# yynps737/zero-latency-yolo

Hardware: AMD Instinct MI355X
Metric: frames_per_sec (higher is better)
Workload: dtype bf16; 1 GPU; YOLOv8-nano 416x416 batch=64 throughput path (BASELINE configs[2]), bf16; engines_per_gpu=3, weights=seeded synthetic (no real weights offline), graph=True, parallelism=single GPU

## Files before the change

zero-latency-yolo_amd/csrc/engine.cpp:

```cpp
#include "zly_internal.h"
#include "weights.h"

#include <algorithm>
#include <atomic>
#include <chrono>
#include <condition_variable>
#include <deque>
#include <map>
#include <mutex>
#include <string>
#include <thread>
#include <type_traits>
#include <vector>
#include <string.h>
#include <stdio.h>
#include <stdlib.h>

namespace zly {

static thread_local std::string g_last_error;

static int fail(int code, const std::string& msg) { g_last_error = msg; return code; }

#define HIP_TRY(expr, code)                                                                        \
// ... 734 lines not shown
    }
    ca.w1 = wb + g.w1; ca.b1 = (const float*)(wb + g.b1); ca.nk1 = g.nk1;
    ca.cat = cb.ptr; ca.cat_cs = cb.C; ca.pair_in_co = e->ops[(size_t)pg.first].in.co; ca.pair_out_co = pg.out.co;
    ca.wA = wb + pg.wA; ca.bA = (const float*)(wb + pg.bA); ca.wB = wb + pg.wB; ca.bB = (const float*)(wb + pg.bB);
    ca.res = g.res;
    ca.w2 = wb + g.w2; ca.b2 = (const float*)(wb + g.b2); ca.nk2 = g.nk2; ca.Cout2 = g.cout2;
    ca.out = ob.ptr; ca.out_cs = ob.C; ca.out_co = g.out.co;
    ca.H = cb.H; ca.W = cb.W; ca.n = n;
    ca.TH = pl.th; ca.TW = pl.tw; ca.tiles_x = pl.tiles_x; ca.tiles_y = pl.tiles_y; ca.total_tiles = pl.total_tiles;
    ca.dump = (e->cfg.flags & ZLY_FLAG_DUMP_LOGITS) ? 1 : 0;
    if (g.c == 64 && g.mid.buf >= 0) { const Buffer& mb = e->bufs[(size_t)g.mid.buf]; ca.mid = mb.ptr; ca.mid_cs = mb.C; }
    return ca;
}

static const std::vector<Launch>& resolve_launches(zly_engine* e, int n)
{
    auto it = e->launches.find(n);
    if (it != e->launches.end()) return it->second;
    const bool bf16 = e->dtype == ZLY_DTYPE_BF16, fusion = bf16 && !(e->cfg.flags & ZLY_FLAG_NO_FUSION), dump = (e->cfg.flags & ZLY_FLAG_DUMP_LOGITS) != 0;
    const int nops = (int)e->ops.size();
    auto c2f_of = [&](const C2fGroup& g, C2fPlan* pl) {
        if (!fusion || e->sw.no_c2f) return false;
        const Buffer& b = e->bufs[(size_t)g.cat];
        return c2f_plan(g.c, g.mode, g.nk1, g.nk2, g.cout2, n, b.H, b.W, e->sw, pl);
    };
    auto pair_of = [&](int a, PairPlan* pl) {
        const Op& A = e->ops[(size_t)a];
        if (A.pair < 0 || !fusion) return false;
        const PairGroup& g = e->pairs[(size_t)A.pair];
        if (g.first != a || !(e->sw.pair_widths & g.c)) return false;
        const Buffer& b = e->bufs[(size_t)A.in.buf];
        return pair_plan(g.c, n, b.H, b.W, e->sw, pl) && pl->total_tiles >= e->sw.pair_min_tiles;
    };
    auto ws_pair_of = [&](int a, WsPairPlan* pl) {
        const Op& A = e->ops[(size_t)a];
        if (A.pair < 0 || !fusion) return false;
        const PairGroup& g = e->pairs[(size_t)A.pair];
        if (g.first != a || g.c != 64 || (e->sw.pair_widths & 64)) return false;
        const ConvArgs ca = make_conv_args(e, A, n), cb = make_conv_args(e, e->ops[(size_t)g.second], n);
        ConvPlan pa{}, pb{};
        conv_plan(e->dtype, 3, ca, e->sw, &pa);
        conv_plan(e->dtype, 3, cb, e->sw, &pb);
        return conv_ws_pair_plan(ca, cb, pa, pb, e->sw, pl);
    };
    bool sppf = fusion && e->sw.sppf_fused && e->sppf_cv1 >= 0;
    if (sppf) {
        const Op& a = e->ops[(size_t)e->sppf_cv1];
// ... 1824 lines not shown
```

zero-latency-yolo_amd/csrc/kernels_pair.hip:

```cpp
#include "zly_internal.h"
#include "conv_device.h"
#include <stdlib.h>
#include <stdio.h>
#include <type_traits>

namespace zly {

typedef __attribute__((ext_vector_type(4))) short s16x4;
typedef __attribute__((ext_vector_type(4))) unsigned int u32x4_t;

template <int C> struct PairGeom;
template <> struct PairGeom<16> {
    static constexpr int CT = 1, KS = 1, FRAGB = 8, PITCH = 48, WTILE = 512;
    static constexpr bool WRES = true;
    typedef s16x4 frag;
    static __device__ __forceinline__ f32x4 mma(frag a, frag b, f32x4 c) { return __builtin_amdgcn_mfma_f32_16x16x16bf16_1k(a, b, c, 0, 0, 0); }
};
template <> struct PairGeom<32> {
    static constexpr int CT = 2, KS = 1, FRAGB = 16, PITCH = 96, WTILE = 1024;
    static constexpr bool WRES = true;
    typedef bf16x8 frag;
    static __device__ __forceinline__ f32x4 mma(frag a, frag b, f32x4 c) { return __builtin_amdgcn_mfma_f32_16x16x32_bf16(a, b, c, 0, 0, 0); }
};
template <> struct PairGeom<64> {
    static constexpr int CT = 4, KS = 2, FRAGB = 16, PITCH = 160, WTILE = 1024;
    static constexpr bool WRES = false;
    typedef bf16x8 frag;
    static __device__ __forceinline__ f32x4 mma(frag a, frag b, f32x4 c) { return __builtin_amdgcn_mfma_f32_16x16x32_bf16(a, b, c, 0, 0, 0); }
};

__device__ __forceinline__ int div_small(int q, float inv) { return (int)(((float)q + 0.5f) * inv); }

template <int C>
__device__ __forceinline__ void pair_taps(const unsigned char* __restrict__ src, const unsigned char* __restrict__ lw, int off, int rowb, int lane,
                                          f32x4 (&acc)[PairGeom<C>::CT])
{
    typedef PairGeom<C> G;
    typedef typename G::frag F;
#pragma unroll
    for (int c = 0; c < G::CT; ++c) acc[c] = f32x4{0.f, 0.f, 0.f, 0.f};
    const unsigned char* wl = lw + lane * G::FRAGB;
    const int kxo[3] = {0, G::FRAGB == 8 ? opaque_offset(G::PITCH) : G::PITCH, G::FRAGB == 8 ? opaque_offset(2 * G::PITCH) : 2 * G::PITCH};
#pragma unroll
    for (int ky = 0; ky < 3; ++ky) {
        const unsigned char* row = src + off + ky * rowb;
#pragma unroll
        for (int kx = 0; kx < 3; ++kx) {
#pragma unroll
            for (int ks = 0; ks < G::KS; ++ks) {
                const F x = *reinterpret_cast<const F*>(row + (G::FRAGB == 8 ? kxo[kx] : kx * G::PITCH) + ks * 64);
#pragma unroll
                for (int c = 0; c < G::CT; ++c) {
                    const F w = *reinterpret_cast<const F*>(wl + ((c * 9 + ky * 3 + kx) * G::KS + ks) * G::WTILE);
                    acc[c] = G::mma(w, x, acc[c]);
// ... 158 lines not shown
                        }
                        store8(dst + g2 * 32 + kq * 8, lo, hi);
                    }
                }
            }
        }
        if (tnext >= a.total_tiles) break;
        tl = tnext;
        __syncthreads();
    }
}

#ifdef ZLY_C2F_DIAG
__device__ unsigned long long* g_c2f_diag = nullptr;
#define C2FSTAMP(k) do { __builtin_amdgcn_sched_barrier(0); unsigned long long t_; asm volatile("s_memtime %0\n\ts_waitcnt lgkmcnt(0)" : "=s"(t_) :: "memory"); dsum[k] += t_ - dT0; dT0 = t_; __builtin_amdgcn_sched_barrier(0); } while (0)
#else
#define C2FSTAMP(k) do { } while (0)
#endif
static constexpr int C2F_BIAS_BYTES = 1024;
static constexpr bool c2f_ring(int c, int mode) { return c == 32 && mode == 3; }
static constexpr bool c2f_y2reg(int c, int mode) { return c == 32 && (mode & 2) != 0; }
static constexpr bool c2f_tight(int c, int nw) { return c == 32 && nw == 16; }
static constexpr int C2F_MAXY = 4;
template <int C, int MODE, int NW, int NLD, int NK1>
__global__ __launch_bounds__(NW * 64) void c2f_kernel(const C2fArgs a)
{
    typedef PairGeom<C> G;
    typedef typename G::frag F;
    constexpr bool FRONT = (MODE & 1) != 0, BACK = (MODE & 2) != 0;
    constexpr bool RING = c2f_ring(C, MODE), Y2REG = c2f_y2reg(C, MODE), TIGHT = c2f_tight(C, NW);
    constexpr int NT = NW * 64;
    constexpr int UPP = C / 8;
    constexpr int WBYTES = 9 * G::CT * G::WTILE;
    constexpr int T1 = 2 * C / 16;
    constexpr int T2MAX = 4;
    extern __shared__ __attribute__((aligned(16))) unsigned char smem[];
#ifdef ZLY_C2F_DIAG
    unsigned long long dsum[12] = {0, 0, 0, 0, 0, 0, 0, 0, 0, 0, 0, 0}, dT0 = __builtin_amdgcn_s_memtime();
    const unsigned long long dstart = dT0;
#endif
    const int PW = a.TW + 4, PH = a.TH + 4, MW = a.TW + 2, MH = a.TH + 2;
    const int w1_bytes = FRONT ? T1 * a.nk1 * 1024 : 0;
    const int T2 = a.Cout2 >> 4;
    const int w2_bytes = BACK ? T2 * a.nk2 * G::WTILE : 0;
    float* lbias = reinterpret_cast<float*>(smem);
    unsigned char* lwA = smem + C2F_BIAS_BYTES;
    unsigned char* lwB = lwA + WBYTES;
    unsigned char* lw1 = lwB + WBYTES;
    unsigned char* lw2 = lw1 + w1_bytes;
    unsigned char* lin = lw2 + w2_bytes;
    unsigned char* lmid = lin + (PH * PW * G::PITCH + 15) / 16 * 16;
    unsigned char* ly2 = lmid + (MH * MW * G::PITCH + 15) / 16 * 16;
    unsigned char* ly0 = ly2 + (BACK && !Y2REG ? (a.TH * a.TW * G::PITCH + 15) / 16 * 16 : 0);

    const int tid = threadIdx.x, lane = tid & 63;
    const int wave = __builtin_amdgcn_readfirstlane(tid >> 6);
    const int p = lane & 15, kq = lane >> 4;
    bf16_t* __restrict__ cat = static_cast<bf16_t*>(a.cat);

    auto stage = [&](unsigned char* dst, const void* src, int bytes) {
        for (int u = tid; u < bytes / 16; u += NT)
            *reinterpret_cast<u32x4_t*>(dst + (size_t)u * 16) = *reinterpret_cast<const u32x4_t*>(static_cast<const unsigned char*>(src) + (size_t)u * 16);
    };
    stage(lwA, a.wA, WBYTES);
    stage(lwB, a.wB, WBYTES);
    if (FRONT) stage(lw1, a.w1, w1_bytes);
    if (BACK) stage(lw2, a.w2, w2_bytes);

    constexpr bool BIAS_LDS = C == 32 && NW == 16;
    if (BIAS_LDS) {
        for (int u = tid; u < C; u += NT) { lbias[u] = a.bA[u]; lbias[C + u] = a.bB[u]; }
        if (FRONT) for (int u = tid; u < 2 * C; u += NT) lbias[2 * C + u] = a.b1[u];
        if (BACK) for (int u = tid; u < a.Cout2; u += NT) lbias[4 * C + u] = a.b2[u];
    }
    constexpr int NBR = BIAS_LDS ? 1 : G::CT, NB1 = BIAS_LDS ? 1 : T1, NB2 = BIAS_LDS ? 1 : T2MAX;
    f32x4 rbA[NBR], rbB[NBR], rb1[NB1], rb2[NB2];
    if (!BIAS_LDS) {
#pragma unroll
        for (int c = 0; c < G::CT; ++c) {
            const int ch = C == 16 ? kq * 4 : (c >> 1) * 32 + kq * 8 + (c & 1) * 4;
            rbA[c % NBR] = *reinterpret_cast<const f32x4*>(a.bA + ch);
// ... 14 lines not shown
            return *reinterpret_cast<const f32x4*>(lbias + base + (c >> 1) * 32 + kq * 8 + (c & 1) * 4);
        }
        return which == 0 ? rbA[c % NBR] : which == 1 ? rbB[c % NBR] : which == 2 ? rb1[c % NB1] : rb2[c % NB2];
    };
    const float invPW = 1.0f / (float)PW, invMW = 1.0f / (float)MW, invTW = 1.0f / (float)a.TW;
    const int tiles_per_img = a.tiles_x * a.tiles_y;
    const int NP0 = PH * PW, NPA = MH * MW, NPB = a.TH * a.TW;
    const int ntA = (NPA + 15) >> 4, ntB = (NPB + 15) >> 4;
    const int NPR = RING ? 4 * PW + 4 * a.TH : 0;
    const int NPI = RING ? NPB : NP0;
    const int ntR = (NPR + 15) >> 4, nt0 = ntR + ((NPI + 15) >> 4);
    const int NPU = NP0 * UPP;

    auto tile_origin = [&](int tl, int& b, int& y0, int& x0) {
        b = tl / tiles_per_img;
        const int r = tl - b * tiles_per_img;
        const int ty = r / a.tiles_x;
        y0 = ty * a.TH; x0 = (r - ty * a.tiles_x) * a.TW;
    };
    auto put_map = [&](unsigned char* dst, const f32x4* o) {
        if (C == 16) store4(reinterpret_cast<bf16_t*>(dst) + kq * 4, o[0]);
        else store8(reinterpret_cast<bf16_t*>(dst) + kq * 8, o[0], o[1]);
    };
    const __amdgpu_buffer_rsrc_t rcat = __builtin_amdgcn_make_buffer_rsrc(a.cat, 0, (unsigned)((size_t)a.n * a.H * a.W * a.cat_cs * 2), 0x00020000);
    auto put_global = [&](int elem, const f32x4* o) {
        if (C == 16) {
            const bf16x4 v = to_bf16x4(o[0]);
            typedef __attribute__((ext_vector_type(2))) unsigned int u32x2_t;
            __builtin_amdgcn_raw_buffer_store_b64(__builtin_bit_cast(u32x2_t, v), rcat, (elem + kq * 4) * 2, 0, 0);
        } else {
            const bf16x8 v = to_bf16x8(o[0], o[1]);
            __builtin_amdgcn_raw_buffer_store_b128(__builtin_bit_cast(u32x4_t, v), rcat, (elem + kq * 8) * 2, 0, 0);
        }
    };

    u32x4_t pre[NLD];
    auto stage_load = [&](int tl) {
        int b, y0, x0;
        tile_origin(tl, b, y0, x0);
        const bf16_t* in = cat + a.pair_in_co;
#pragma unroll
        for (int i = 0; i < NLD; ++i) {
            const int u = tid + i * NT;
            u32x4_t v = {0u, 0u, 0u, 0u};
            if (u < NPU) {
                const int px = u / UPP, part = u - px * UPP;
                const int py = div_small(px, invPW), pxx = px - py * PW;
                const int gy = y0 - 2 + py, gx = x0 - 2 + pxx;
                if ((unsigned)gy < (unsigned)a.H && (unsigned)gx < (unsigned)a.W)
                    v = *reinterpret_cast<const u32x4_t*>(in + ((size_t)(b * a.H + gy) * a.W + gx) * a.cat_cs + part * 8);
            }
            pre[i] = v;
        }
    };
    auto stage_store = [&]() {
#pragma unroll
        for (int i = 0; i < NLD; ++i) {
            const int u = tid + i * NT;
            if (u < NPU) {
                const int px = u / UPP, part = u - px * UPP;
                *reinterpret_cast<u32x4_t*>(lin + px * G::PITCH + part * 16) = pre[i];
            }
        }
    };

    int tl = blockIdx.x;
    if (tl >= a.total_tiles) return;
    if (!FRONT) stage_load(tl);
    C2FSTAMP(0);
    while (true) {
        int b, y0, x0;
        tile_origin(tl, b, y0, x0);
        const int tnext = tl + gridDim.x;
        if (!FRONT) {
            stage_store();
            __syncthreads();
            C2FSTAMP(1);
            if (tnext < a.total_tiles) stage_load(tnext);
        } else {
            const int pF = TIGHT ? opaque_offset(p) : p, kqF = TIGHT ? opaque_offset(kq) : kq, laneF = TIGHT ? opaque_offset(lane) : lane;
            const bf16_t* __restrict__ xa = static_cast<const bf16_t*>(a.x) + a.x_co;
            const bf16_t* __restrict__ xb = static_cast<const bf16_t*>(a.x2) + a.x2_co;
            const bool dual = a.x2 != nullptr;
            const unsigned char* w1l = lw1 + laneF * 16;
            auto cv1_pixel = [&](int t, int& py, int& px) -> bool {
                if (RING && t < ntR) {
                    const int q = t * 16 + pF, r = min(q, NPR - 1);
                    if (r < 4 * PW) {
                        const int row = div_small(r, invPW);
                        px = r - row * PW; py = row < 2 ? row : row + a.TH;
                    } else {
                        const int s = r - 4 * PW, col = s & 3;
                        py = 2 + (s >> 2); px = col < 2 ? col : col + a.TW;
                    }
                    return q < NPR;
                }
                const int q = (t - ntR) * 16 + pF, j = min(q, NPI - 1);
                if (RING) {
                    const int iy = div_small(j, invTW);
                    py = iy + 2; px = j - iy * a.TW + 2;
                } else {
                    py = div_small(j, invPW); px = j - py * PW;
                }
                return q < NPI;
            };
            auto load_x = [&](int t, bf16x8 (&xf)[NK1]) {
                int py, px;
                cv1_pixel(t, py, px);
                const int gy = y0 - 2 + py, gx = x0 - 2 + px;
                const bool inimg = (unsigned)gy < (unsigned)a.H && (unsigned)gx < (unsigned)a.W;
                const size_t pa = dual ? ((size_t)(b * (a.H >> 1) + (gy >> 1)) * (a.W >> 1) + (gx >> 1)) * a.x_cs : ((size_t)(b * a.H + gy) * a.W + gx) * a.x_cs;
                const size_t pb2 = ((size_t)(b * a.H + gy) * a.W + gx) * a.x2_cs;
#pragma unroll
                for (int s = 0; s < NK1; ++s) {
                    const int ci = s * 32 + kqF * 8;
#pragma unroll
                    for (int j = 0; j < 8; ++j) xf[s][j] = (bf16_t)0.0f;
                    if (inimg) xf[s] = (dual && ci >= a.split_c) ? *reinterpret_cast<const bf16x8*>(xb + pb2 + (ci - a.split_c)) : *reinterpret_cast<const bf16x8*>(xa + pa + ci);
                }
            };
            bf16x8 xcur[NK1], xnext[NK1];
            if (wave < nt0) load_x(wave, xcur);
            __syncthreads();
            C2FSTAMP(1);
            auto cv1_tile = [&](auto c0, int t) {
                constexpr int C0 = decltype(c0)::value;
                f32x4 acc[T1];
#pragma unroll
                for (int c = C0; c < T1; ++c) acc[c] = f32x4{0.f, 0.f, 0.f, 0.f};
#pragma unroll
                for (int s = 0; s < NK1; ++s)
#pragma unroll
                    for (int c = C0; c < T1; ++c) {
                        const bf16x8 wf = *reinterpret_cast<const bf16x8*>(w1l + (c * NK1 + s) * 1024);
                        acc[c] = __builtin_amdgcn_mfma_f32_16x16x32_bf16(wf, xcur[s], acc[c], 0, 0, 0);
                    }
#pragma unroll
                for (int s = 0; s < NK1; ++s) xcur[s] = xnext[s];
                int py, px;
                const bool valid = cv1_pixel(t, py, px);
                const int gy = y0 - 2 + py, gx = x0 - 2 + px;
                const bool inimg = (unsigned)gy < (unsigned)a.H && (unsigned)gx < (unsigned)a.W;
                f32x4 o[T1];
#pragma unroll
                for (int c = C0; c < T1; ++c) {
                    f32x4 v = acc[c] + bias_of(2, c);
#pragma unroll
                    for (int r = 0; r < 4; ++r) v[r] = inimg ? silu<bf16_t>(v[r]) : 0.0f;
                    o[c] = v;
                }
                if (valid) {
                    put_map(lin + (size_t)(py * PW + px) * G::PITCH, o + G::CT);
                    if (C0 == 0 && inimg && (RING || ((unsigned)(py - 2) < (unsigned)a.TH && (unsigned)(px - 2) < (unsigned)a.TW))) {
                        if (MODE == 3) put_map(ly0 + (size_t)((py - 2) * a.TW + px - 2) * G::PITCH, o);
                        if (MODE == 1 || a.dump) {
                            const int dst = ((b * a.H + gy) * a.W + gx) * a.cat_cs;
                            put_global(dst, o);
                            put_global(dst + C, o + G::CT);
                        }
                    }
                }
            };
            for (int t = wave; t < nt0; t += NW) {
                if (t + NW < nt0) load_x(t + NW, xnext);
                if (RING && t < ntR) cv1_tile(std::integral_constant<int, G::CT>(), t);
                else cv1_tile(std::integral_constant<int, 0>(), t);
            }
            C2FSTAMP(2);
            __syncthreads();
            C2FSTAMP(3);
        }

        const int pA = TIGHT ? opaque_offset(p) : p, kqA = TIGHT ? opaque_offset(kq) : kq, laneA = TIGHT ? opaque_offset(lane) : lane;
        for (int t = wave; t < ntA; t += NW) {
            const int q = t * 16 + pA;
            const int qc = min(q, NPA - 1);
            const int my = div_small(qc, invMW), mx = qc - my * MW;
            f32x4 acc[G::CT];
            pair_taps<C>(lin, lwA, (my * PW + mx) * G::PITCH + kqA * G::FRAGB, PW * G::PITCH, laneA, acc);
            const int gy = y0 - 1 + my, gx = x0 - 1 + mx;
            const bool inimg = (unsigned)gy < (unsigned)a.H && (unsigned)gx < (unsigned)a.W;
            f32x4 o[G::CT];
#pragma unroll
            for (int c = 0; c < G::CT; ++c) {
                f32x4 v = acc[c] + bias_of(0, c);
#pragma unroll
                for (int r = 0; r < 4; ++r) v[r] = inimg ? silu<bf16_t>(v[r]) : 0.0f;
                o[c] = v;
            }
            if (q < NPA) put_map(lmid + (size_t)(my * MW + mx) * G::PITCH, o);
        }
        C2FSTAMP(4);
        __syncthreads();
        C2FSTAMP(5);

        constexpr int NS = MODE == 2 ? 4 : 3;
        const int pB = TIGHT ? opaque_offset(p) : p, kqB = TIGHT ? opaque_offset(kq) : kq, laneB = TIGHT ? opaque_offset(lane) : lane;
        constexpr int NY = Y2REG ? C2F_MAXY : 1;
        F y2f[NY], xs2[NS - 1], xs2n[NS - 1];
#pragma unroll
        for (int i = 0; i < NY; ++i) y2f[i] = F{};
#pragma unroll
        for (int s = 0; s < NS - 1; ++s) xs2n[s] = F{};
        auto y2_put = [&](int i, F v) {
            static_assert(C2F_MAXY == 4, "one branch per carried tile");
            if (i == 0) y2f[0] = v; else if (i == 1) y2f[1 % NY] = v; else if (i == 2) y2f[2 % NY] = v; else y2f[3 % NY] = v;
        };
        auto y2_get = [&](int i) -> F { return i == 0 ? y2f[0] : i == 1 ? y2f[1 % NY] : i == 2 ? y2f[2 % NY] : y2f[3 % NY]; };
        auto load_cv2 = [&](int t, F (&x)[NS - 1]) {
            const int qc = min(t * 16 + pB, NPB - 1);
            const int oy = div_small(qc, invTW), ox = qc - oy * a.TW;
            if (MODE == 2) {
                const int gy = min(y0 + oy, a.H - 1), gx = min(x0 + ox, a.W - 1);
                const bf16_t* gp = cat + ((size_t)(b * a.H + gy) * a.W + gx) * a.cat_cs + kqB * (G::FRAGB / 2);
                x[0] = *reinterpret_cast<const F*>(gp);
                x[1] = *reinterpret_cast<const F*>(gp + C);
            } else {
                x[0] = *reinterpret_cast<const F*>(ly0 + (size_t)qc * G::PITCH + kqB * G::FRAGB);
            }
            x[NS - 2] = *reinterpret_cast<const F*>(lin + (size_t)((oy + 2) * PW + ox + 2) * G::PITCH + kqB * G::FRAGB);
        };
        if (Y2REG) load_cv2(wave, xs2);
        auto conv_b_tile = [&](int t, int i) {
            if (BACK && TIGHT) asm volatile("" ::: "memory");
            const int q = t * 16 + pB;
            const int qc = min(q, NPB - 1);
            const int oy = div_small(qc, invTW), ox = qc - oy * a.TW;
            f32x4 acc[G::CT];
            pair_taps<C>(lmid, lwB, (oy * MW + ox) * G::PITCH + kqB * G::FRAGB, MW * G::PITCH, laneB, acc);
            f32x4 o[G::CT];
#pragma unroll
            for (int c = 0; c < G::CT; ++c) {
                f32x4 v = acc[c] + bias_of(1, c);
#pragma unroll
                for (int r = 0; r < 4; ++r) v[r] = silu<bf16_t>(v[r]);
                o[c] = v;
            }
            const int gy = y0 + oy, gx = x0 + ox;
            if (a.res) {
                const unsigned char* xs = lin + ((oy + 2) * PW + ox + 2) * G::PITCH;
                if (C == 16) o[0] += load4(reinterpret_cast<const bf16_t*>(xs) + kqB * 4);
                else { f32x4 ra, rb; load8(reinterpret_cast<const bf16_t*>(xs) + kqB * 8, ra, rb); o[0] += ra; o[1 % G::CT] += rb; }
            }
            if constexpr (Y2REG) {
                if constexpr (C == 16) y2_put(i, __builtin_bit_cast(F, to_bf16x4(o[0])));
                else y2_put(i, __builtin_bit_cast(F, to_bf16x8(o[0], o[1 % G::CT])));
            } else if (BACK && q < NPB) put_map(ly2 + (size_t)qc * G::PITCH, o);
            if ((!BACK || a.dump) && q < NPB && gy < a.H && gx < a.W)
                put_global(((b * a.H + gy) * a.W + gx) * a.cat_cs + a.pair_out_co, o);
        };
        for (int t = wave, i = 0; t < ntB; t += NW, ++i) conv_b_tile(t, i);

        C2FSTAMP(6);
        if (BACK) {
            if (!Y2REG) __syncthreads();
            C2FSTAMP(7);
            const unsigned char* w2l = lw2 + laneB * G::FRAGB;
            for (int t = wave, i = 0; t < ntB; t += NW, ++i) {
                if (!Y2REG) load_cv2(t, xs2);
                else if (t + NW < ntB) load_cv2(t + NW, xs2n);
                const int q = t * 16 + pB;
                const int qc = min(q, NPB - 1);
                const F yf = Y2REG ? y2_get(i) : *reinterpret_cast<const F*>(ly2 + (size_t)qc * G::PITCH + kqB * G::FRAGB);
                const int oy = div_small(qc, invTW), ox = qc - oy * a.TW;
                const int gy = min(y0 + oy, a.H - 1), gx = min(x0 + ox, a.W - 1);
                f32x4 acc[T2MAX];
#pragma unroll
                for (int c = 0; c < T2MAX; ++c) acc[c] = f32x4{0.f, 0.f, 0.f, 0.f};
#pragma unroll
                for (int s = 0; s < NS; ++s)
#pragma unroll
                    for (int c = 0; c < T2MAX; ++c)
                        if (c < T2) acc[c] = G::mma(*reinterpret_cast<const F*>(w2l + (c * NS + s) * G::WTILE), s < NS - 1 ? xs2[s < NS - 1 ? s : 0] : yf, acc[c]);
                if (Y2REG) {
#pragma unroll
                    for (int s = 0; s < NS - 1; ++s) xs2[s] = xs2n[s];
                }
                if (q < NPB && y0 + oy < a.H && x0 + ox < a.W) {
                    bf16_t* dst = static_cast<bf16_t*>(a.out) + ((size_t)(b * a.H + gy) * a.W + gx) * a.out_cs + a.out_co;
#pragma unroll
                    for (int g2 = 0; g2 < T2MAX / 2; ++g2) {
                        if (2 * g2 >= T2) break;
                        f32x4 lo = acc[2 * g2] + bias_of(3, 2 * g2), hi = acc[2 * g2 + 1] + bias_of(3, 2 * g2 + 1);
#pragma unroll
                        for (int r = 0; r < 4; ++r) { lo[r] = silu<bf16_t>(lo[r]); hi[r] = silu<bf16_t>(hi[r]); }
                        store8(dst + g2 * 32 + kqB * 8, lo, hi);
                    }
                }
            }
        }
        C2FSTAMP(8);
        if (tnext >= a.total_tiles) break;
        tl = tnext;
        if (!FRONT) __syncthreads();
    }
#ifdef ZLY_C2F_DIAG
    if (lane == 0 && g_c2f_diag) {
        unsigned long long* o = g_c2f_diag + ((size_t)blockIdx.x * NW + wave) * 16;
        for (int i = 0; i < 9; ++i) o[i] = dsum[i];
        o[9] = __builtin_amdgcn_s_memtime() - dstart;
    }
#endif
}

static constexpr int PAIR_NW16 = 16, PAIR_NW32 = 8, PAIR_NW64 = 8, PAIR_NLD = 4, PAIR_NLD64 = 6;
static int pair_nw(int c) { return c == 16 ? PAIR_NW16 : PAIR_NW32; }
static int pair_nld(int c) { return c == 64 ? PAIR_NLD64 : PAIR_NLD; }
static constexpr int PAIR_LDS_MAX = 160 * 1024;

// ... 39 lines not shown
}

static constexpr int C2F_NW16 = 16, C2F_NW32 = 8, C2F_NLD = 4;
static int c2f_nw32(int mode, const Switches& sw)
{
    if (sw.c2f32_nw == 8 || sw.c2f32_nw == 16) return sw.c2f32_nw;
    return mode == 1 ? C2F_NW32 : 16;
}
static size_t c2f_lds_bytes(int c, int mode, int nk1, int nk2, int cout2, int th, int tw)
{
    const size_t pitch = (size_t)pair_pitch(c), wtile = c == 16 ? 512 : 1024, ct = c / 16;
    size_t b = C2F_BIAS_BYTES + 2 * 9 * ct * wtile;
    if (mode & 1) b += (size_t)(2 * c / 16) * nk1 * 1024;
    if (mode & 2) b += (size_t)(cout2 / 16) * nk2 * wtile;
    b += ((size_t)(th + 4) * (tw + 4) * pitch + 15) / 16 * 16 + ((size_t)(th + 2) * (tw + 2) * pitch + 15) / 16 * 16;
    if ((mode & 2) && !c2f_y2reg(c, mode)) b += ((size_t)th * tw * pitch + 15) / 16 * 16;
    if (mode == 3) b += ((size_t)th * tw * pitch + 15) / 16 * 16;
    return b;
}

typedef void (*c2f_fn)(const C2fArgs);
static c2f_fn pick_c2f(int c, int mode, int nk1, int nw32);

bool c2f_plan(int c, int mode, int nk1, int nk2, int cout2, int n, int H, int W, const Switches& sw, C2fPlan* plan)
{
    if (c == 64 && mode >= 1 && mode <= 3) return c2f64_plan(mode, nk1, nk2, cout2, n, H, W, sw, plan);
    if ((c != 16 && c != 32) || mode < 1 || mode > 3 || !pick_c2f(c, mode, nk1, c2f_nw32(mode, sw))) return false;
    if ((mode & 2) && nk2 != (mode == 2 ? 4 : 3)) return false;
    const int ncu = sw.num_cus, nw = c == 16 ? C2F_NW16 : c2f_nw32(mode, sw);
    const size_t lds_cap = sw.c2f_lds_kb ? (size_t)sw.c2f_lds_kb * 1024 : (size_t)PAIR_LDS_MAX;
    double best = 1e30;
    for (int th = 4; th <= 32; ++th) {
        for (int tw = 8; tw <= 64; ++tw) {
            if (c2f_lds_bytes(c, mode, nk1, nk2, cout2, th, tw) > lds_cap) continue;
            if (sw.c2f_tile_th && (sw.c2f_tile_th != th || sw.c2f_tile_tw != tw)) continue;
            if (!(mode & 1) && (th + 4) * (tw + 4) * (c / 8) > nw * 64 * C2F_NLD) continue;
            if (c2f_y2reg(c, mode) && (th * tw + 15) / 16 > nw * C2F_MAXY) continue;
            const int tx = (W + tw - 1) / tw, ty = (H + th - 1) / th;
            const long tiles = (long)n * tx * ty;
            const long rounds = (tiles + ncu - 1) / ncu;
            const bool ring = c2f_ring(c, mode);
            const int ntR = ring ? (4 * (tw + 4) + 4 * th + 15) / 16 : 0, nt1 = ((ring ? th * tw : (th + 4) * (tw + 4)) + 15) / 16, ntA = ((th + 2) * (tw + 2) + 15) / 16, ntB = (th * tw + 15) / 16;
            const int ct = c / 16;
            const double w_cv1 = (double)(2 * ct * nk1 + 2.0 * 2 * ct) / (9.0 * ct + 2.0 * ct);
            const double w_cv2 = (double)((cout2 / 16) * nk2 + 2.0 * (cout2 / 16)) / (9.0 * ct + 2.0 * ct);
            double per_tile = (double)((ntA + nw - 1) / nw + (ntB + nw - 1) / nw) + 1.5 * 16 / nw;
            if (mode & 1) {
                const int ring0 = (ntR + nw - 1) / nw, all0 = (ntR + nt1 + nw - 1) / nw;
                per_tile += w_cv1 * (0.5 * ring0 + (all0 - ring0));
            }
// ... 21 lines not shown
    return c == 16 ? pick_c2f_c<16, C2F_NW16>(mode, nk1) : nw32 == 16 ? pick_c2f_c<32, 16>(mode, nk1) : pick_c2f_c<32, C2F_NW32>(mode, nk1);
}

hipError_t c2f_init()
{
    static const int nk1s[3] = {1, 2, 6};
    for (int c = 16; c <= 32; c += 16)
        for (int mode = 1; mode <= 3; ++mode)
            for (int i = 0; i < 3; ++i)
                for (int nw32 = 8; nw32 <= 16; nw32 += 8) {
                    hipError_t r = hipFuncSetAttribute((const void*)pick_c2f(c, mode, nk1s[i], nw32), hipFuncAttributeMaxDynamicSharedMemorySize, PAIR_LDS_MAX);
                    if (r != hipSuccess) return r;
                }
    return c2f64_init();
}

hipError_t launch_c2f(int c, int mode, const C2fArgs& a, const C2fPlan& plan, hipStream_t s)
{
    if (c == 64) return launch_c2f64(mode, a, plan, s);
    if ((c != 16 && c != 32) || mode < 1 || mode > 3 || a.TH != plan.th || a.TW != plan.tw || plan.grid < 1) return hipErrorInvalidValue;
    if (a.cat_cs % 8 || a.pair_in_co % c || a.pair_out_co % c || a.out_cs % 8 || a.out_co % 8) return hipErrorInvalidValue;
    if ((mode & 1) && (a.x_cs % 8 || a.x_co % 8 || (a.x2 && (a.x2_cs % 8 || a.x2_co % 8 || a.split_c % 32 || (a.H & 1) || (a.W & 1))))) return hipErrorInvalidValue;
    if ((mode & 2) && (a.Cout2 % 32 || a.Cout2 > 64)) return hipErrorInvalidValue;
    const int nw = c == 16 ? C2F_NW16 : plan.nw;
    if (c == 32 && nw != 8 && nw != 16) return hipErrorInvalidValue;
    if (c2f_y2reg(c, mode) && (a.TH * a.TW + 15) / 16 > nw * C2F_MAXY) return hipErrorInvalidValue;
    c2f_fn fn = pick_c2f(c, mode, a.nk1, nw);
    if (!fn || (mode == 2 && a.pair_in_co != 2 * c)) return hipErrorInvalidValue;
    hipLaunchKernelGGL(fn, dim3((unsigned)plan.grid), dim3(nw * 64), (size_t)plan.lds_bytes, s, a);
    return hipGetLastError();
}

hipError_t launch_pair(int c, const PairArgs& a, const PairPlan& plan, hipStream_t s)
{
    if ((c != 16 && c != 32 && c != 64) || a.TH != plan.th || a.TW != plan.tw || plan.grid < 1) return hipErrorInvalidValue;
    if (a.in_cs % 8 || a.in_co % 8 || a.out_cs % 8 || a.out_co % 8) return hipErrorInvalidValue;
    if (c == 16) hipLaunchKernelGGL((bottleneck_pair_kernel<16, PAIR_NW16, PAIR_NLD>), dim3((unsigned)plan.grid), dim3(PAIR_NW16 * 64), (size_t)plan.lds_bytes, s, a);
    else if (c == 32) hipLaunchKernelGGL((bottleneck_pair_kernel<32, PAIR_NW32, PAIR_NLD>), dim3((unsigned)plan.grid), dim3(PAIR_NW32 * 64), (size_t)plan.lds_bytes, s, a);
    else         hipLaunchKernelGGL((bottleneck_pair_kernel<64, PAIR_NW64, PAIR_NLD64>), dim3((unsigned)plan.grid), dim3(PAIR_NW64 * 64), (size_t)plan.lds_bytes, s, a);
    return hipGetLastError();
}

}
```

zero-latency-yolo_amd/csrc/zly_internal.h:

```cpp
#pragma once
#include <hip/hip_runtime.h>
#include <stdint.h>
#include <stddef.h>
#include <string>
#include "zly.h"
#include "front_variants.h"

namespace zly {

typedef __bf16 bf16_t;

struct FrameDesc {
    unsigned long long src_off;
    int w, h;
};
#define ZLY_DESC_FMT_SHIFT 56
__host__ __device__ __forceinline__ unsigned long long desc_pack(unsigned long long off, int fmt) { return off | ((unsigned long long)fmt << ZLY_DESC_FMT_SHIFT); }
__host__ __device__ __forceinline__ unsigned long long desc_off(unsigned long long v) { return v & ((1ull << ZLY_DESC_FMT_SHIFT) - 1); }
__host__ __device__ __forceinline__ int desc_fmt(unsigned long long v) { return (int)(v >> ZLY_DESC_FMT_SHIFT); }

__host__ __device__ __forceinline__ int front_level(int fmt)
{
    return fmt == ZLY_PIX_BGR ? ZLY_FRONT_BGR : fmt >= ZLY_PIX_NV12_BT601 && fmt <= ZLY_PIX_I420_BT709 ? ZLY_FRONT_YUV : ZLY_FRONT_PACKED;
}
// ... 138 lines not shown
    int TH, TW, tiles_x, tiles_y, total_tiles;
    int res;
};
struct PairPlan { int th, tw, tiles_x, tiles_y, total_tiles, grid, lds_bytes; };
bool       pair_plan(int c, int n, int H, int W, const Switches& sw, PairPlan* plan);
hipError_t pair_init();
hipError_t launch_pair(int c, const PairArgs& a, const PairPlan& plan, hipStream_t s);

struct C2fArgs {
    const void* x;  int x_cs, x_co;
    const void* x2; int x2_cs, x2_co, split_c;
    const void* w1; const float* b1; int nk1;
    void* cat; int cat_cs;
    int pair_in_co, pair_out_co;
    const void* wA; const float* bA; const void* wB; const float* bB; int res;
    const void* w2; const float* b2; int nk2, Cout2;
    void* out; int out_cs, out_co;
    int H, W, n;
    int TH, TW, tiles_x, tiles_y, total_tiles;
    int dump;
    void* mid; int mid_cs;
};
struct C2fPlan { int th, tw, tiles_x, tiles_y, total_tiles, grid, lds_bytes, nw; };
bool       c2f_plan(int c, int mode, int nk1, int nk2, int cout2, int n, int H, int W, const Switches& sw, C2fPlan* plan);
hipError_t c2f_init();
hipError_t launch_c2f(int c, int mode, const C2fArgs& a, const C2fPlan& plan, hipStream_t s);
bool       c2f64_plan(int mode, int nk1, int nk2, int cout2, int n, int H, int W, const Switches& sw, C2fPlan* plan);
hipError_t c2f64_init();
hipError_t launch_c2f64(int mode, const C2fArgs& a, const C2fPlan& plan, hipStream_t s);

hipError_t launch_preprocess(int dtype, const uint8_t* src, const FrameDesc* desc, int n,
                             void* out_nhwc8, float* out_nchw_f32, int tw, int th, hipStream_t s, FrontVariant v);
hipError_t launch_nchw_to_nhwc8(int dtype, const float* in_nchw, void* out_nhwc8, int n, int tw, int th, hipStream_t s);
hipError_t launch_sppf_pool(int dtype, void* buf, int cs, int c, int n, int H, int W, hipStream_t s, int six_pass = 0);
bool       sppf_pool16_ok(int dtype, int cs, int c, int n, int H, int W, int six_pass);
hipError_t launch_tap_to_nchw(int dtype, const void* in, int cs, int co, int C, int H, int W, int idx, float* out, hipStream_t s);

struct StemArgs {
    const uint8_t* src; const FrameDesc* desc;
    const void* wgt; const float* bias;
    void* out; int out_cs, out_co;
    int tw, th, Ho, Wo, Cout, tiles_x;
};
hipError_t launch_stem_fused(const StemArgs& a, int n, hipStream_t s, FrontVariant v);
int stem_tiles_x(int Wo);
struct Stem1Args {
    StemArgs st;
// ... 70 lines not shown
```

Baseline: 117,300 frames/s.

## Use 32-bit buffer addressing and carry pixel coordinates in fused C2f kernel

Replaces 64-bit pointer arithmetic in the fused C2f kernel with raw buffer loads and stores using 32-bit (often 24-bit multiply) offsets, and precomputes local and global pixel indices once per cv1 tile in a struct. For c=16 the computed pixel coordinates are carried from the prefetch step instead of being recomputed. The aim is to cut VALU address math and register pressure. A host-side check now rejects fusion when tensors exceed 4 GiB so 32-bit offsets stay valid.

After: 117,700 frames/s (median of 6 runs). Within noise of the previous version (+0.3%).

```diff
diff --git a/zero-latency-yolo_amd/csrc/engine.cpp b/zero-latency-yolo_amd/csrc/engine.cpp
--- a/zero-latency-yolo_amd/csrc/engine.cpp
+++ b/zero-latency-yolo_amd/csrc/engine.cpp
@@ -780,7 +780,9 @@
     auto c2f_of = [&](const C2fGroup& g, C2fPlan* pl) {
         if (!fusion || e->sw.no_c2f) return false;
         const Buffer& b = e->bufs[(size_t)g.cat];
-        return c2f_plan(g.c, g.mode, g.nk1, g.nk2, g.cout2, n, b.H, b.W, e->sw, pl);
+        int max_cs = b.C;
+        for (int v : {g.x.buf, g.x2.buf, g.out.buf}) if (v >= 0 && e->bufs[(size_t)v].C > max_cs) max_cs = e->bufs[(size_t)v].C;
+        return c2f_plan(g.c, g.mode, g.nk1, g.nk2, g.cout2, n, b.H, b.W, e->sw, pl, max_cs);
     };
     auto pair_of = [&](int a, PairPlan* pl) {
         const Op& A = e->ops[(size_t)a];
diff --git a/zero-latency-yolo_amd/csrc/kernels_pair.hip b/zero-latency-yolo_amd/csrc/kernels_pair.hip
--- a/zero-latency-yolo_amd/csrc/kernels_pair.hip
+++ b/zero-latency-yolo_amd/csrc/kernels_pair.hip
@@ -30,6 +30,7 @@
 };
 
 __device__ __forceinline__ int div_small(int q, float inv) { return (int)(((float)q + 0.5f) * inv); }
+__device__ __forceinline__ int mul32(int a, int b) { int r = a * b; asm("" : "+v"(r)); return r; }
 
 template <int C>
 __device__ __forceinline__ void pair_taps(const unsigned char* __restrict__ src, const unsigned char* __restrict__ lw, int off, int rowb, int lane,
@@ -234,13 +235,17 @@
 static constexpr bool c2f_y2reg(int c, int mode) { return c == 32 && (mode & 2) != 0; }
 static constexpr bool c2f_tight(int c, int nw) { return c == 32 && nw == 16; }
 static constexpr int C2F_MAXY = 4;
+static constexpr bool c2f_carry(int c) { return c == 16; }
+static constexpr bool c2f_xbuf(int c, int mode, int nw) { return !(c == 32 && mode == 1 && nw == 8); }
+struct Cv1Px { int lpix, ypix, gy, gx, gpix; bool valid, inimg; };
+static constexpr unsigned long long C2F_MAX_TENSOR_BYTES = 1ull << 32;
 template <int C, int MODE, int NW, int NLD, int NK1>
 __global__ __launch_bounds__(NW * 64) void c2f_kernel(const C2fArgs a)
 {
     typedef PairGeom<C> G;
     typedef typename G::frag F;
     constexpr bool FRONT = (MODE & 1) != 0, BACK = (MODE & 2) != 0;
-    constexpr bool RING = c2f_ring(C, MODE), Y2REG = c2f_y2reg(C, MODE), TIGHT = c2f_tight(C, NW);
+    constexpr bool RING = c2f_ring(C, MODE), Y2REG = c2f_y2reg(C, MODE), TIGHT = c2f_tight(C, NW), CARRY = c2f_carry(C), XBUF = c2f_xbuf(C, MODE, NW);
     constexpr int NT = NW * 64;
     constexpr int UPP = C / 8;
     constexpr int WBYTES = 9 * G::CT * G::WTILE;
@@ -268,7 +273,6 @@
     const int tid = threadIdx.x, lane = tid & 63;
     const int wave = __builtin_amdgcn_readfirstlane(tid >> 6);
     const int p = lane & 15, kq = lane >> 4;
-    bf16_t* __restrict__ cat = static_cast<bf16_t*>(a.cat);
 
     auto stage = [&](unsigned char* dst, const void* src, int bytes) {
         for (int u = tid; u < bytes / 16; u += NT)
@@ -329,7 +333,8 @@
         if (C == 16) store4(reinterpret_cast<bf16_t*>(dst) + kq * 4, o[0]);
         else store8(reinterpret_cast<bf16_t*>(dst) + kq * 8, o[0], o[1]);
     };
-    const __amdgpu_buffer_rsrc_t rcat = __builtin_amdgcn_make_buffer_rsrc(a.cat, 0, (unsigned)((size_t)a.n * a.H * a.W * a.cat_cs * 2), 0x00020000);
+    const unsigned map_px = (unsigned)a.n * a.H * a.W;
+    const __amdgpu_buffer_rsrc_t rcat = __builtin_amdgcn_make_buffer_rsrc(a.cat, 0, map_px * a.cat_cs * 2, 0x00020000);
     auto put_global = [&](int elem, const f32x4* o) {
         if (C == 16) {
             const bf16x4 v = to_bf16x4(o[0]);
@@ -341,21 +346,28 @@
         }
     };
 
+    const __amdgpu_buffer_rsrc_t rout = __builtin_amdgcn_make_buffer_rsrc(a.out, 0, BACK ? map_px * a.out_cs * 2 : 0u, 0x00020000);
+    auto ld_frag = [&](__amdgpu_buffer_rsrc_t r, int off) -> F {
+        typedef __attribute__((ext_vector_type(2))) unsigned int u32x2_t;
+        if constexpr (sizeof(F) == 8) return __builtin_bit_cast(F, (u32x2_t)__builtin_amdgcn_raw_buffer_load_b64(r, off, 0, 0));
+        else return __builtin_bit_cast(F, (u32x4_t)__builtin_amdgcn_raw_buffer_load_b128(r, off, 0, 0));
+    };
+
     u32x4_t pre[NLD];
     auto stage_load = [&](int tl) {
         int b, y0, x0;
         tile_origin(tl, b, y0, x0);
-        const bf16_t* in = cat + a.pair_in_co;
+        const int bpx = b * a.H * a.W;
 #pragma unroll
         for (int i = 0; i < NLD; ++i) {
             const int u = tid + i * NT;
             u32x4_t v = {0u, 0u, 0u, 0u};
             if (u < NPU) {
                 const int px = u / UPP, part = u - px * UPP;
-                const int py = div_small(px, invPW), pxx = px - py * PW;
+                const int py = div_small(px, invPW), pxx = px - __mul24(py, PW);
                 const int gy = y0 - 2 + py, gx = x0 - 2 + pxx;
                 if ((unsigned)gy < (unsigned)a.H && (unsigned)gx < (unsigned)a.W)
-                    v = *reinterpret_cast<const u32x4_t*>(in + ((size_t)(b * a.H + gy) * a.W + gx) * a.cat_cs + part * 8);
+                    v = __builtin_amdgcn_raw_buffer_load_b128(rcat, mul32(bpx + __mul24(gy, a.W) + gx, a.cat_cs * 2) + (a.pair_in_co + part * 8) * 2, 0, 0);
             }
             pre[i] = v;
         }
@@ -378,6 +390,7 @@
     while (true) {
         int b, y0, x0;
         tile_origin(tl, b, y0, x0);
+        const int imgpx = b * a.H * a.W;
         const int tnext = tl + gridDim.x;
         if (!FRONT) {
             stage_store();
@@ -386,48 +399,81 @@
             if (tnext < a.total_tiles) stage_load(tnext);
         } else {
             const int pF = TIGHT ? opaque_offset(p) : p, kqF = TIGHT ? opaque_offset(kq) : kq, laneF = TIGHT ? opaque_offset(lane) : lane;
-            const bf16_t* __restrict__ xa = static_cast<const bf16_t*>(a.x) + a.x_co;
-            const bf16_t* __restrict__ xb = static_cast<const bf16_t*>(a.x2) + a.x2_co;
-            const bool dual = a.x2 != nullptr;
+            const bool dual = NK1 > 1 && a.x2 != nullptr;
+            const int split = dual ? a.split_c : (1 << 30);
+            const __amdgpu_buffer_rsrc_t rxa = __builtin_amdgcn_make_buffer_rsrc(const_cast<void*>(a.x), 0, 0xffffffffu, 0x00020000);
+            const __amdgpu_buffer_rsrc_t rxb = __builtin_amdgcn_make_buffer_rsrc(const_cast<void*>(dual ? a.x2 : a.x), 0, 0xffffffffu, 0x00020000);
+            const unsigned xa_lane = (unsigned)(a.x_co + kqF * 8) * 2, xb_lane = (unsigned)(a.x2_co + kqF * 8) * 2;
             const unsigned char* w1l = lw1 + laneF * 16;
-            auto cv1_pixel = [&](int t, int& py, int& px) -> bool {
+            auto cv1_pixel = [&](int t) -> Cv1Px {
+                Cv1Px c;
+                int py, px;
                 if (RING && t < ntR) {
                     const int q = t * 16 + pF, r = min(q, NPR - 1);
                     if (r < 4 * PW) {
                         const int row = div_small(r, invPW);
-                        px = r - row * PW; py = row < 2 ? row : row + a.TH;
+                        px = r - __mul24(row, PW); py = row < 2 ? row : row + a.TH;
+                        c.lpix = row < 2 ? r : r + a.TH * PW;
                     } else {
                         const int s = r - 4 * PW, col = s & 3;
                         py = 2 + (s >> 2); px = col < 2 ? col : col + a.TW;
+                        c.lpix = __mul24(py, PW) + px;
                     }
-                    return q < NPR;
-                }
-                const int q = (t - ntR) * 16 + pF, j = min(q, NPI - 1);
-                if (RING) {
-                    const int iy = div_small(j, invTW);
-                    py = iy + 2; px = j - iy * a.TW + 2;
+                    c.valid = q < NPR;
+                    c.ypix = 0;
                 } else {
-                    py = div_small(j, invPW); px = j - py * PW;
-                }
-                return q < NPI;
+                    const int q = (t - ntR) * 16 + pF, j = min(q, NPI - 1);
+                    if (RING) {
+                        const int iy = div_small(j, invTW);
+                        py = iy + 2; px = j - __mul24(iy, a.TW) + 2;
+                        c.lpix = j + 4 * iy + (2 * PW + 2); c.ypix = j;
+                    } else {
+                        py = div_small(j, invPW); px = j - __mul24(py, PW);
+                        c.lpix = j; c.ypix = j - 4 * py - (2 * a.TW + 2);
+                    }
+                    c.valid = q < NPI;
+                }
+                c.gy = y0 - 2 + py; c.gx = x0 - 2 + px;
+                c.inimg = (unsigned)c.gy < (unsigned)a.H && (unsigned)c.gx < (unsigned)a.W;
+                if (!(c.inimg && (RING || ((unsigned)(py - 2) < (unsigned)a.TH && (unsigned)(px - 2) < (unsigned)a.TW)))) c.ypix = -1;
+                c.gpix = imgpx + __mul24(c.gy, a.W) + c.gx;
+                return c;
             };
-            auto load_x = [&](int t, bf16x8 (&xf)[NK1]) {
-                int py, px;
-                cv1_pixel(t, py, px);
-                const int gy = y0 - 2 + py, gx = x0 - 2 + px;
-                const bool inimg = (unsigned)gy < (unsigned)a.H && (unsigned)gx < (unsigned)a.W;
-                const size_t pa = dual ? ((size_t)(b * (a.H >> 1) + (gy >> 1)) * (a.W >> 1) + (gx >> 1)) * a.x_cs : ((size_t)(b * a.H + gy) * a.W + gx) * a.x_cs;
-                const size_t pb2 = ((size_t)(b * a.H + gy) * a.W + gx) * a.x2_cs;
+            auto load_x = [&](int t, bf16x8 (&xf)[NK1]) -> Cv1Px {
+                const Cv1Px c = cv1_pixel(t);
+                if (!XBUF) {
+                    const bf16_t* __restrict__ xa = static_cast<const bf16_t*>(a.x) + a.x_co;
+                    const bf16_t* __restrict__ xb = static_cast<const bf16_t*>(a.x2) + a.x2_co;
+                    const size_t pa = dual ? ((size_t)(b * (a.H >> 1) + (c.gy >> 1)) * (a.W >> 1) + (c.gx >> 1)) * a.x_cs : (size_t)c.gpix * a.x_cs;
+                    const size_t pb2 = (size_t)c.gpix * a.x2_cs;
+#pragma unroll
+                    for (int s = 0; s < NK1; ++s) {
+                        const int ci = s * 32 + kqF * 8;
+#pragma unroll
+                        for (int j = 0; j < 8; ++j) xf[s][j] = (bf16_t)0.0f;
+                        if (c.inimg) xf[s] = (dual && ci >= a.split_c) ? *reinterpret_cast<const bf16x8*>(xb + pb2 + (ci - a.split_c)) : *reinterpret_cast<const bf16x8*>(xa + pa + ci);
+                    }
+                    return c;
+                }
+                unsigned pa, pb2;
+                if (dual) {
+                    const int hpix = __mul24(__mul24(b, a.H >> 1) + (c.gy >> 1), a.W >> 1) + (c.gx >> 1);
+                    pa = mul32(c.inimg ? hpix : 0, a.x_cs * 2) + xa_lane;
+                    pb2 = mul32(c.inimg ? c.gpix : 0, a.x2_cs * 2) + xb_lane;
+                } else {
+                    pa = pb2 = mul32(c.inimg ? c.gpix : 0, a.x_cs * 2) + xa_lane;
+                }
 #pragma unroll
                 for (int s = 0; s < NK1; ++s) {
-                    const int ci = s * 32 + kqF * 8;
-#pragma unroll
-                    for (int j = 0; j < 8; ++j) xf[s][j] = (bf16_t)0.0f;
-                    if (inimg) xf[s] = (dual && ci >= a.split_c) ? *reinterpret_cast<const bf16x8*>(xb + pb2 + (ci - a.split_c)) : *reinterpret_cast<const bf16x8*>(xa + pa + ci);
-                }
+                    const int ci = s * 32;
+                    const bool second = ci >= split;
+                    xf[s] = __builtin_bit_cast(bf16x8, __builtin_amdgcn_raw_buffer_load_b128(second ? rxb : rxa, (int)(second ? pb2 : pa), second ? (ci - split) * 2 : ci * 2, 0));
+                }
+                return c;
             };
             bf16x8 xcur[NK1], xnext[NK1];
-            if (wave < nt0) load_x(wave, xcur);
+            Cv1Px ccur = {}, cnext = {};
+            if (wave < nt0) ccur = load_x(wave, xcur);
             __syncthreads();
             C2FSTAMP(1);
             auto cv1_tile = [&](auto c0, int t) {
@@ -444,10 +490,15 @@
                     }
 #pragma unroll
                 for (int s = 0; s < NK1; ++s) xcur[s] = xnext[s];
-                int py, px;
-                const bool valid = cv1_pixel(t, py, px);
-                const int gy = y0 - 2 + py, gx = x0 - 2 + px;
-                const bool inimg = (unsigned)gy < (unsigned)a.H && (unsigned)gx < (unsigned)a.W;
+                Cv1Px c1 = CARRY ? ccur : cv1_pixel(t);
+                ccur = cnext;
+                if (CARRY) {
+                    const bool ring = RING && t < ntR;
+                    const int q = (ring ? t : t - ntR) * 16 + pF, j = min(q, NPI - 1);
+                    c1.valid = q < (ring ? NPR : NPI);
+                    if (RING) c1.ypix = c1.inimg ? j : -1; else c1.lpix = j;
+                }
+                const bool inimg = c1.inimg;
                 f32x4 o[T1];
 #pragma unroll
                 for (int c = C0; c < T1; ++c) {
@@ -456,12 +507,12 @@
                     for (int r = 0; r < 4; ++r) v[r] = inimg ? silu<bf16_t>(v[r]) : 0.0f;
                     o[c] = v;
                 }
-                if (valid) {
-                    put_map(lin + (size_t)(py * PW + px) * G::PITCH, o + G::CT);
-                    if (C0 == 0 && inimg && (RING || ((unsigned)(py - 2) < (unsigned)a.TH && (unsigned)(px - 2) < (unsigned)a.TW))) {
-                        if (MODE == 3) put_map(ly0 + (size_t)((py - 2) * a.TW + px - 2) * G::PITCH, o);
+                if (c1.valid) {
+                    put_map(lin + __umul24(c1.lpix, G::PITCH), o + G::CT);
+                    if (C0 == 0 && c1.ypix >= 0) {
+                        if (MODE == 3) put_map(ly0 + __umul24(c1.ypix, G::PITCH), o);
                         if (MODE == 1 || a.dump) {
-                            const int dst = ((b * a.H + gy) * a.W + gx) * a.cat_cs;
+                            const int dst = mul32(MODE == 1 ? c1.gpix : cv1_pixel(t).gpix, a.cat_cs);
                             put_global(dst, o);
                             put_global(dst + C, o + G::CT);
                         }
@@ -469,7 +520,7 @@
                 }
             };
             for (int t = wave; t < nt0; t += NW) {
-                if (t + NW < nt0) load_x(t + NW, xnext);
+                if (t + NW < nt0) cnext = load_x(t + NW, xnext);
                 if (RING && t < ntR) cv1_tile(std::integral_constant<int, G::CT>(), t);
                 else cv1_tile(std::integral_constant<int, 0>(), t);
             }
@@ -482,9 +533,9 @@
         for (int t = wave; t < ntA; t += NW) {
             const int q = t * 16 + pA;
             const int qc = min(q, NPA - 1);
-            const int my = div_small(qc, invMW), mx = qc - my * MW;
+            const int my = div_small(qc, invMW), mx = qc - __mul24(my, MW);
             f32x4 acc[G::CT];
-            pair_taps<C>(lin, lwA, (my * PW + mx) * G::PITCH + kqA * G::FRAGB, PW * G::PITCH, laneA, acc);
+            pair_taps<C>(lin, lwA, __mul24(qc + 2 * my, G::PITCH) + kqA * G::FRAGB, PW * G::PITCH, laneA, acc);
             const int gy = y0 - 1 + my, gx = x0 - 1 + mx;
             const bool inimg = (unsigned)gy < (unsigned)a.H && (unsigned)gx < (unsigned)a.W;
             f32x4 o[G::CT];
@@ -495,7 +546,7 @@
                 for (int r = 0; r < 4; ++r) v[r] = inimg ? silu<bf16_t>(v[r]) : 0.0f;
                 o[c] = v;
             }
-            if (q < NPA) put_map(lmid + (size_t)(my * MW + mx) * G::PITCH, o);
+            if (q < NPA) put_map(lmid + __umul24(qc, G::PITCH), o);
         }
         C2FSTAMP(4);
         __syncthreads();
@@ -516,25 +567,25 @@
         auto y2_get = [&](int i) -> F { return i == 0 ? y2f[0] : i == 1 ? y2f[1 % NY] : i == 2 ? y2f[2 % NY] : y2f[3 % NY]; };
         auto load_cv2 = [&](int t, F (&x)[NS - 1]) {
             const int qc = min(t * 16 + pB, NPB - 1);
-            const int oy = div_small(qc, invTW), ox = qc - oy * a.TW;
+            const int oy = div_small(qc, invTW), ox = qc - __mul24(oy, a.TW);
             if (MODE == 2) {
                 const int gy = min(y0 + oy, a.H - 1), gx = min(x0 + ox, a.W - 1);
-                const bf16_t* gp = cat + ((size_t)(b * a.H + gy) * a.W + gx) * a.cat_cs + kqB * (G::FRAGB / 2);
-                x[0] = *reinterpret_cast<const F*>(gp);
-                x[1] = *reinterpret_cast<const F*>(gp + C);
+                const int go = mul32(imgpx + __mul24(gy, a.W) + gx, a.cat_cs * 2) + kqB * G::FRAGB;
+                x[0] = ld_frag(rcat, go);
+                x[1] = ld_frag(rcat, go + C * 2);
             } else {
-                x[0] = *reinterpret_cast<const F*>(ly0 + (size_t)qc * G::PITCH + kqB * G::FRAGB);
-            }
-            x[NS - 2] = *reinterpret_cast<const F*>(lin + (size_t)((oy + 2) * PW + ox + 2) * G::PITCH + kqB * G::FRAGB);
+                x[0] = *reinterpret_cast<const F*>(ly0 + __umul24(qc, G::PITCH) + kqB * G::FRAGB);
+            }
+            x[NS - 2] = *reinterpret_cast<const F*>(lin + __umul24(qc + 4 * oy + (2 * PW + 2), G::PITCH) + kqB * G::FRAGB);
         };
         if (Y2REG) load_cv2(wave, xs2);
         auto conv_b_tile = [&](int t, int i) {
             if (BACK && TIGHT) asm volatile("" ::: "memory");
             const int q = t * 16 + pB;
             const int qc = min(q, NPB - 1);
-            const int oy = div_small(qc, invTW), ox = qc - oy * a.TW;
+            const int oy = div_small(qc, invTW), ox = qc - __mul24(oy, a.TW);
             f32x4 acc[G::CT];
-            pair_taps<C>(lmid, lwB, (oy * MW + ox) * G::PITCH + kqB * G::FRAGB, MW * G::PITCH, laneB, acc);
+            pair_taps<C>(lmid, lwB, __mul24(qc + 2 * oy, G::PITCH) + kqB * G::FRAGB, MW * G::PITCH, laneB, acc);
             f32x4 o[G::CT];
 #pragma unroll
             for (int c = 0; c < G::CT; ++c) {
@@ -545,16 +596,16 @@
             }
             const int gy = y0 + oy, gx = x0 + ox;
             if (a.res) {
-                const unsigned char* xs = lin + ((oy + 2) * PW + ox + 2) * G::PITCH;
+                const unsigned char* xs = lin + __umul24(qc + 4 * oy + (2 * PW + 2), G::PITCH);
                 if (C == 16) o[0] += load4(reinterpret_cast<const bf16_t*>(xs) + kqB * 4);
                 else { f32x4 ra, rb; load8(reinterpret_cast<const bf16_t*>(xs) + kqB * 8, ra, rb); o[0] += ra; o[1 % G::CT] += rb; }
             }
             if constexpr (Y2REG) {
                 if constexpr (C == 16) y2_put(i, __builtin_bit_cast(F, to_bf16x4(o[0])));
                 else y2_put(i, __builtin_bit_cast(F, to_bf16x8(o[0], o[1 % G::CT])));
-            } else if (BACK && q < NPB) put_map(ly2 + (size_t)qc * G::PITCH, o);
+            } else if (BACK && q < NPB) put_map(ly2 + __umul24(qc, G::PITCH), o);
             if ((!BACK || a.dump) && q < NPB && gy < a.H && gx < a.W)
-                put_global(((b * a.H + gy) * a.W + gx) * a.cat_cs + a.pair_out_co, o);
+                put_global(mul32(imgpx + __mul24(gy, a.W) + gx, a.cat_cs) + a.pair_out_co, o);
         };
         for (int t = wave, i = 0; t < ntB; t += NW, ++i) conv_b_tile(t, i);
 
@@ -568,9 +619,9 @@
                 else if (t + NW < ntB) load_cv2(t + NW, xs2n);
                 const int q = t * 16 + pB;
                 const int qc = min(q, NPB - 1);
-                const F yf = Y2REG ? y2_get(i) : *reinterpret_cast<const F*>(ly2 + (size_t)qc * G::PITCH + kqB * G::FRAGB);
-                const int oy = div_small(qc, invTW), ox = qc - oy * a.TW;
-                const int gy = min(y0 + oy, a.H - 1), gx = min(x0 + ox, a.W - 1);
+                const F yf = Y2REG ? y2_get(i) : *reinterpret_cast<const F*>(ly2 + __umul24(qc, G::PITCH) + kqB * G::FRAGB);
+                const int oy = div_small(qc, invTW), ox = qc - __mul24(oy, a.TW);
+                const int gy = y0 + oy, gx = x0 + ox;
                 f32x4 acc[T2MAX];
 #pragma unroll
                 for (int c = 0; c < T2MAX; ++c) acc[c] = f32x4{0.f, 0.f, 0.f, 0.f};
@@ -583,15 +634,15 @@
 #pragma unroll
                     for (int s = 0; s < NS - 1; ++s) xs2[s] = xs2n[s];
                 }
-                if (q < NPB && y0 + oy < a.H && x0 + ox < a.W) {
-                    bf16_t* dst = static_cast<bf16_t*>(a.out) + ((size_t)(b * a.H + gy) * a.W + gx) * a.out_cs + a.out_co;
+                if (q < NPB && gy < a.H && gx < a.W) {
+                    const int dst = mul32(imgpx + __mul24(gy, a.W) + gx, a.out_cs * 2) + (a.out_co + kqB * 8) * 2;
 #pragma unroll
                     for (int g2 = 0; g2 < T2MAX / 2; ++g2) {
                         if (2 * g2 >= T2) break;
                         f32x4 lo = acc[2 * g2] + bias_of(3, 2 * g2), hi = acc[2 * g2 + 1] + bias_of(3, 2 * g2 + 1);
 #pragma unroll
                         for (int r = 0; r < 4; ++r) { lo[r] = silu<bf16_t>(lo[r]); hi[r] = silu<bf16_t>(hi[r]); }
-                        store8(dst + g2 * 32 + kqB * 8, lo, hi);
+                        __builtin_amdgcn_raw_buffer_store_b128(__builtin_bit_cast(u32x4_t, to_bf16x8(lo, hi)), rout, dst + g2 * 64, 0, 0);
                     }
                 }
             }
@@ -677,10 +728,21 @@
 typedef void (*c2f_fn)(const C2fArgs);
 static c2f_fn pick_c2f(int c, int mode, int nk1, int nw32);
 
-bool c2f_plan(int c, int mode, int nk1, int nk2, int cout2, int n, int H, int W, const Switches& sw, C2fPlan* plan)
+bool c2f_tensors_fit(int c, int mode, int nk1, int cout2, int n, int H, int W, int max_cs)
+{
+    if (n < 1 || H < 1 || W < 1 || H >= (1 << 23) || W >= (1 << 23)) return false;
+    int cs = max_cs > 0 ? max_cs : c * (mode == 3 ? 3 : 4);
+    if (max_cs <= 0 && (mode & 1) && nk1 * 32 > cs) cs = nk1 * 32;
+    if (max_cs <= 0 && (mode & 2) && cout2 > cs) cs = cout2;
+    const unsigned long long rows = (unsigned long long)n * H, row_bytes = (unsigned long long)W * cs * 2;
+    return rows <= C2F_MAX_TENSOR_BYTES / row_bytes && rows * row_bytes < C2F_MAX_TENSOR_BYTES;
+}
+
+bool c2f_plan(int c, int mode, int nk1, int nk2, int cout2, int n, int H, int W, const Switches& sw, C2fPlan* plan, int max_cs)
 {
     if (c == 64 && mode >= 1 && mode <= 3) return c2f64_plan(mode, nk1, nk2, cout2, n, H, W, sw, plan);
     if ((c != 16 && c != 32) || mode < 1 || mode > 3 || !pick_c2f(c, mode, nk1, c2f_nw32(mode, sw))) return false;
+    if (!c2f_tensors_fit(c, mode, nk1, cout2, n, H, W, max_cs)) return false;
     if ((mode & 2) && nk2 != (mode == 2 ? 4 : 3)) return false;
     const int ncu = sw.num_cus, nw = c == 16 ? C2F_NW16 : c2f_nw32(mode, sw);
     const size_t lds_cap = sw.c2f_lds_kb ? (size_t)sw.c2f_lds_kb * 1024 : (size_t)PAIR_LDS_MAX;
@@ -748,6 +810,12 @@
     if (a.cat_cs % 8 || a.pair_in_co % c || a.pair_out_co % c || a.out_cs % 8 || a.out_co % 8) return hipErrorInvalidValue;
     if ((mode & 1) && (a.x_cs % 8 || a.x_co % 8 || (a.x2 && (a.x2_cs % 8 || a.x2_co % 8 || a.split_c % 32 || (a.H & 1) || (a.W & 1))))) return hipErrorInvalidValue;
     if ((mode & 2) && (a.Cout2 % 32 || a.Cout2 > 64)) return hipErrorInvalidValue;
+    if ((mode & 1) && a.x2 && (a.nk1 < 2 || a.split_c < 32 || a.split_c >= a.nk1 * 32)) return hipErrorInvalidValue;
+    int max_cs = a.cat_cs;
+    if ((mode & 1) && a.x_cs > max_cs) max_cs = a.x_cs;
+    if ((mode & 1) && a.x2 && a.x2_cs > max_cs) max_cs = a.x2_cs;
+    if ((mode & 2) && a.out_cs > max_cs) max_cs = a.out_cs;
+    if (!c2f_tensors_fit(c, mode, a.nk1, a.Cout2, a.n, a.H, a.W, max_cs)) return hipErrorInvalidValue;
     const int nw = c == 16 ? C2F_NW16 : plan.nw;
     if (c == 32 && nw != 8 && nw != 16) return hipErrorInvalidValue;
     if (c2f_y2reg(c, mode) && (a.TH * a.TW + 15) / 16 > nw * C2F_MAXY) return hipErrorInvalidValue;
diff --git a/zero-latency-yolo_amd/csrc/zly_internal.h b/zero-latency-yolo_amd/csrc/zly_internal.h
--- a/zero-latency-yolo_amd/csrc/zly_internal.h
+++ b/zero-latency-yolo_amd/csrc/zly_internal.h
@@ -184,7 +184,8 @@
     void* mid; int mid_cs;
 };
 struct C2fPlan { int th, tw, tiles_x, tiles_y, total_tiles, grid, lds_bytes, nw; };
-bool       c2f_plan(int c, int mode, int nk1, int nk2, int cout2, int n, int H, int W, const Switches& sw, C2fPlan* plan);
+bool       c2f_plan(int c, int mode, int nk1, int nk2, int cout2, int n, int H, int W, const Switches& sw, C2fPlan* plan, int max_cs = 0);
+bool       c2f_tensors_fit(int c, int mode, int nk1, int cout2, int n, int H, int W, int max_cs);
 hipError_t c2f_init();
 hipError_t launch_c2f(int c, int mode, const C2fArgs& a, const C2fPlan& plan, hipStream_t s);
 bool       c2f64_plan(int mode, int nk1, int nk2, int cout2, int n, int H, int W, const Switches& sw, C2fPlan* plan);
```
